# kalj/dealii-cuda

Measured on AMD Instinct MI355X. Metric: DoFs/s on 1305x Laplace vmult (bmop), p=4 3D uniform, higher is better.
Workload: dtype f64; 1 GPU; bmop: DEGREE_FE=4, DIMENSION=3, MATRIX_FREE_UNIFORM_MESH, hyper_cube(-1,1), 54^3 cells, 10218313 DoFs, 1 z-slab(s); cells_per_dir=54, n_dofs=10218313, n_cells=157464, parallelism=slab1, dof_numbering=caller's (lexicographic), finite=True, clock_ramp_steps=2000

## Files before the change

dealii-cuda_amd/csrc/mfgpu_api.hip:

```cpp
#include <hip/hip_runtime.h>

#include <type_traits>

#include <algorithm>
#include <cmath>
#include <cstdlib>
#include <cstring>
#include <memory>
#include <string>
#include <vector>

#include "mfgpu_kernels.h"

using namespace mfgpu;

struct EventTimer {
  std::vector<Event> ev;
  size_t used = 0;
  double ms = 0.0;
  int begin(hipStream_t st) {
    if (used + 2 > ev.size()) {
      Event e0, e1;
      int rc;
      if ((rc = e0.create(hipEventDefault)) || (rc = e1.create(hipEventDefault))) return rc;
// ... 49 lines not shown
  DeviceArray<uint32_t> d_cell_batch, d_cell_pos;
  size_t n_plane_cells = 0;
  DeviceArray<uint32_t> d_cmask, d_orphans;
  DeviceArray<void> d_hnw;
  DeviceArray<uint32_t> d_constrained;
  uint32_t n_constrained = 0;
  DeviceArray<void> d_tabsd;
  DeviceArray<void> d_tab2;
  bool twopass = true;
  DeviceArray<uint32_t> d_batch_nint, d_halo_off;
  std::vector<uint32_t> seg_end;
  std::vector<DeviceArray<uint32_t>> d_p2arr, d_p2tiles;
  std::vector<uint32_t> n_p2tiles;
  DeviceArray<uint32_t> d_p2rec, d_p2tab;
  bool p2_shared = false, p2_reverse = false, no_shared_records = false;
  Stream side;
  std::vector<Event> ev_seg;
  Event ev_side;
  bool side_pending = false;
  DeviceArray<void> d_halo;
  DeviceArray<unsigned long long> d_stamps;
  size_t lds = 0, device_bytes = 0;
  PlaneKernel planes = PlaneKernel::none;
  BatchKernel batches = BatchKernel::none;
  enum { kPlain, kMasked, kBatch };
  CellKernel<double> kernels_f64[3];
  CellKernel<float> kernels_f32[3];
  template <typename T>
  CellKernel<T> &kernel(int which) {
    if constexpr (std::is_same<T, double>::value) return kernels_f64[which];
// ... 61 lines not shown
        const double s = 0.5 * (S[r * n + c] + S[r2 * n + c2]);
        S[r * n + c] = S[r2 * n + c2] = s;
        const double d = 0.5 * (Dt[r * n + c] - Dt[r2 * n + c2]);
        Dt[r * n + c] = d;
        Dt[r2 * n + c2] = -d;
      } else if (r == r2 && c == c2) {
        Dt[r * n + c] = 0.0;
      }
    }
  return 0;
}

int upload_pass2(mfgpu_handle *h, const uint32_t *priority, uint32_t n_priority) {
  const Plan &P = h->plan;
  const size_t ng = 1 + h->seg_end.size();
  const bool shared = P.sh_p2_use && !h->no_shared_records && n_priority == 0 && ng == 2;
  std::vector<Pass2Group> groups;
  int rc;
  if ((rc = pass2_groups(P, h->seg_end, priority, n_priority, shared, groups))) return rc;
  std::vector<DeviceArray<uint32_t>> d_arr(ng), d_tiles(ng);
  std::vector<uint32_t> n_tiles(ng, 0u);
  const bool reverse = (size_t)P.halo_off.back() * esize(h->number_type) <= ((size_t)256 << 20);
  DeviceArray<uint32_t> d_rec, d_tab;
  if (shared) {
    if ((rc = d_rec.upload(P.sh_p2rec.data(), P.sh_p2rec.size()))) return rc;
    if ((rc = d_tab.upload(P.sh_p2tab.data(), P.sh_p2tab.size()))) return rc;
  }
  for (size_t g = 0; g < ng; ++g) {
    std::vector<uint32_t> arr, tiles;
    build_pass2_classes(groups[g].dofs, groups[g].offsets, groups[g].slots, arr, tiles);
    n_tiles[g] = (uint32_t)(tiles.size() / 4);
    if (reverse) {
      const size_t nt = tiles.size() / 4;
      for (size_t a = 0, b = nt ? nt - 1 : 0; a < b; ++a, --b)
        for (int w = 0; w < 4; ++w) std::swap(tiles[4 * a + w], tiles[4 * b + w]);
    }
    if ((rc = d_arr[g].upload(arr.data(), arr.size()))) return rc;
    if ((rc = d_tiles[g].upload(tiles.data(), tiles.size()))) return rc;
  }
  h->d_p2arr = std::move(d_arr);
  h->d_p2tiles = std::move(d_tiles);
// ... 567 lines not shown
  const bool hn = (d.flags & MFGPU_HANGING_NODES) != 0;
  if (hn && (!d.constraint_mask || !d.constraint_weights)) {
    set_error("MFGPU_HANGING_NODES needs constraint_mask and constraint_weights");
    return MFGPU_EINVAL;
  }
  std::unique_ptr<mfgpu_handle, decltype(&mfgpu_destroy)> h(new mfgpu_handle(), mfgpu_destroy);
  int rc = choose_kernel_and_plan(d, h->planes, h->batches, h->plan);
  if (rc) return rc;
  h->dim = d.dim;
  h->n = d.degree + 1;
  h->nd = h->plan.nd;
  h->number_type = d.number_type;
  h->hn = hn;
  h->twopass = !(d.flags & MFGPU_COLORED_SCATTER);
  h->no_shared_records = (d.flags & MFGPU_NO_SHARED_RECORDS) != 0;
  h->updatable = (d.flags & MFGPU_UPDATABLE_COEFFICIENTS) != 0;
  const int nn = h->n * h->n;
  std::vector<double> sv(nn), sg(nn);
  for (int i = 0; i < nn; ++i) {
    sv[i] = d.number_type == MFGPU_F64 ? ((const double *)d.shape_values)[i] : ((const float *)d.shape_values)[i];
    sg[i] = d.number_type == MFGPU_F64 ? ((const double *)d.shape_gradients)[i] : ((const float *)d.shape_gradients)[i];
  }
  h->sv = sv;
  h->sg = sg;
  rc = derive_tables(h->n, sv.data(), sg.data(), h->S, h->Dt);
  if (!rc) rc = check_symmetrize(h->n, h->S, h->Dt);
  if (!rc) rc = d.number_type == MFGPU_F64 ? create_typed<double>(h.get(), d) : create_typed<float>(h.get(), d);
  if (!rc && d.n_constrained) {
    h->n_constrained = d.n_constrained;
    rc = h->d_constrained.upload(d.constrained_dofs, d.n_constrained);
// ... 105 lines not shown
  if (h->twopass) {
    const uint32_t nb = (uint32_t)s[0], npl = P.n_plane_batches, nplain = P.n_plain_plane_batches;
    const uint32_t edge[4] = {0u, nplain, npl, nb};
    s[1] = 0;
    for (size_t g = 0; g < h->seg_end.size(); ++g) {
      const uint32_t s0 = g ? h->seg_end[g - 1] : 0u, s1 = h->seg_end[g];
      for (int f = 0; f < 3; ++f)
        if (std::max(s0, edge[f]) < std::min(s1, edge[f + 1])) ++s[1];
    }
    s[6] = P.sdofs.size();
    s[7] = P.halo_off.back();
  }
  return 0;
}

int mfgpu_record_stats(const mfgpu_handle *h, uint64_t s[4]) {
  if (!h || !s) return MFGPU_EINVAL;
  const Plan &P = h->plan;
  const size_t n = (size_t)P.n, nb = (size_t)p_kgu((int)n) * 64, nx = ((n * n + 1) / 2) * (p_cells_per_wave((int)n) * n);
  const bool planes = h->planes != PlaneKernel::none;
  s[0] = (h->shared_records ? 1 : 0) | (h->p2_shared ? 2 : 0);
  s[1] = planes ? P.sh_dofs.size() / nb : 0;
  s[2] = planes ? P.sh_idx.size() / nx : 0;
  s[3] = h->record_bytes;
  return 0;
}

const char *mfgpu_kernel_name(const mfgpu_handle *h) {
  if (!h) return "";
  const bool x = h->batches == BatchKernel::x;
// ... 149 lines not shown
```

dealii-cuda_amd/csrc/mfgpu_internal.h:

```cpp
#ifndef MFGPU_INTERNAL_H
#define MFGPU_INTERNAL_H

#include <cstdint>
#include <string>
#include <vector>

#include "../../include/mfgpu.h"

namespace mfgpu {

void set_error(const std::string &msg);

inline int ipow(int a, int e) {
  int r = 1;
  for (int i = 0; i < e; ++i) r *= a;
  return r;
}

constexpr int p_cells_per_wave(int n) { return 64 / n; }
constexpr int p_ji(int n) { return n == 3 ? 2 : n == 4 ? 5 : n == 5 ? 9 : n == 6 ? 14 : 23; }
constexpr int p_hs(int n) { return n == 3 ? 3 : n == 4 ? 6 : n == 5 ? 9 : n == 6 ? 14 : 18; }
constexpr int p_kgu(int n) { return p_ji(n) + p_hs(n); }
constexpr int p_cell_stride(int n) {
  int s = n * n * n;
// ... 34 lines not shown
  std::vector<uint32_t> orphans;
  std::vector<uint32_t> batch_nint;
  std::vector<uint32_t> halo_off;
  std::vector<uint32_t> sdofs;
  std::vector<uint32_t> s_off;
  std::vector<uint32_t> s_idx;
  std::vector<uint32_t> chunks;
  std::vector<uint32_t> gstarts;
  uint32_t max_batch_dofs = 0, max_batch_cells = 0;
  uint32_t n_plane_batches = 0;
  uint32_t n_plain_plane_batches = 0;
  std::vector<uint32_t> pr_dofs, pr_idx, pr_hn, pr_hn_slot;
  std::vector<uint32_t> sh_dofs, sh_idx, sh_batch;
  bool sh_use = false;
  std::vector<uint32_t> sh_p2rec, sh_p2tab;
  bool sh_p2_use = false;
  uint64_t n_first = 0, n_add = 0;
};

struct PlanLimits {
  uint32_t max_cells = 0, max_dofs = 0;
  uint32_t interior_max = 0, shared_max = 0, halo_stride = 0;
  bool segregate_masked = false;
  bool masked_planes = false;
  uint32_t private_max = 0;
};

int build_plan(const mfgpu_desc &d, Plan &plan, uint32_t max_chunks = 3, const PlanLimits *limits = nullptr);

struct HnLine {
// ... 17 lines not shown
}
constexpr bool kernel_exists(BatchKernel k, int n, int , bool , bool sh, bool ) {
  return k != BatchKernel::none && n >= 2 && n <= 7 && !sh;
}
constexpr int kFusedWidths[] = {3, 2};
constexpr bool fused_kernel_exists(BatchKernel k, int n, int number_type, bool hn, bool , int nv) {
  return k == BatchKernel::g && n >= 2 && n <= 7 && (nv == 2 || nv == 3) &&
         !(hn && number_type == MFGPU_F64 && n >= (nv == 3 ? 6 : 7));
}
std::vector<uint32_t> multi_groups(uint32_t n_vectors, const std::vector<uint32_t> &widths);
int build_plane_records(Plan &plan, const uint32_t *constraint_mask);
constexpr int kShBatchWords = 4;
constexpr double kShareMaxFraction = 0.5;
void share_plane_records(Plan &plan);
constexpr int kP2Header = 16, kP2MaxK = 12, kP2SlotBits = 12;
void share_pass2_records(Plan &plan);

std::vector<uint16_t> x_lane_permutation(int n);
std::vector<uint16_t> x_pencil_runs(const std::vector<uint16_t> &lmap, int n);
struct Pass2Group {
  std::vector<uint32_t> dofs, offsets = std::vector<uint32_t>(1, 0u), slots;
};
int pass2_groups(const Plan &plan, const std::vector<uint32_t> &seg_end, const uint32_t *priority, uint32_t n_priority,
                 bool shared, std::vector<Pass2Group> &groups);

int derive_tables(int n, const double *shape_values, const double *shape_gradients,
                  std::vector<double> &S, std::vector<double> &Dt);

int handle_number_type(const mfgpu_handle *h);
int handle_set_priority_dofs(mfgpu_handle *h, const uint32_t *ids, uint32_t n);
// ... 20 lines not shown
```

dealii-cuda_amd/csrc/mfgpu_kernels.h:

```cpp
#ifndef MFGPU_KERNELS_H
#define MFGPU_KERNELS_H

#include <hip/hip_runtime.h>

#include <type_traits>

#include "mfgpu_device.h"
#include "mfgpu_internal.h"

namespace mfgpu {

template <typename T>
struct ApplyArgs {
  const uint32_t *batch_cell_off;
  const uint32_t *batch_dof_off;
  const uint32_t *bdofs;
  const uint8_t *bflags;
  const uint16_t *lmap;
  const uint16_t *lmapx;
  const uint16_t *perm;
  const uint32_t *bdofsp;
  const uint32_t *idxp;
  const T *coefp;
  const uint32_t *hnrec;
// ... 106 lines not shown
#undef MFGPU_CELL_LOOP_FAMILY
template <typename T>
using MultiKernel = CellKernel<T, MultiArgs<T>>;
template <typename T, typename Args>
hipError_t g_bind_width(int n, bool hn, bool sh, bool mass, int nv, uint32_t nb_max, CellKernel<T, Args> *k);

void build_pass2_classes(const std::vector<uint32_t> &sdofs, const std::vector<uint32_t> &s_off,
                         const std::vector<uint32_t> &s_idx, std::vector<uint32_t> &arr, std::vector<uint32_t> &tiles);
template <typename T>
hipError_t reduce_classes_launch(T *dst, const T *src, const T *halo, const uint32_t *arr, const uint32_t *tiles,
                                 uint32_t n_tiles, int add, hipStream_t st);
template <typename T>
hipError_t reduce_classes_multi_launch(int nv, T *dst, const T *src, size_t stride, T *const *halos, const uint32_t *arr,
                                       const uint32_t *tiles, uint32_t n_tiles, int add, hipStream_t st);
template <typename T>
hipError_t reduce_owner_batches_launch(T *dst, const T *src, const T *halo, const uint32_t *rec, const uint32_t *tab,
                                       uint32_t n_batches, uint32_t hstride, int reverse, int add, hipStream_t st);
template <typename T>
hipError_t relayout_coef_launch(T *out, const T *in, const uint32_t *cell_batch, const uint32_t *cell_pos,
                                size_t total, int n, hipStream_t st);
template <typename T>
hipError_t fold_general_launch(T *M, const T *coef, const T *jxw, const T *jinv, const uint32_t *order,
                               uint32_t n_cells, uint32_t nd, hipStream_t st);
template <typename T>
hipError_t fold_general2_launch(T *M, const T *coef, const T *jxw, const T *jinv, const uint32_t *order,
                                uint32_t n_cells, uint32_t nd, hipStream_t st);
template <typename T>
hipError_t orphan_launch(T *dst, const T *src, const uint32_t *orph, uint32_t n, int add, hipStream_t st);
template <typename T>
hipError_t coefficient_launch(T *coef, const T *qpts, size_t nq, int dim, hipStream_t st);
template <typename T>
// ... 70 lines not shown
```

dealii-cuda_amd/csrc/mfgpu_pass2.hip:

```cpp
#include <hip/hip_runtime.h>

#include <algorithm>

#include "mfgpu_kernels.h"

namespace mfgpu {

namespace {

template <typename T>
struct GroupHalos {
  size_t stride;
  const T *h[kMaxFusedWidth];
};
template <typename T, typename P>
__device__ __forceinline__ P *vec_at(const T *, P *p, int) { return p; }
template <typename T, typename P>
__device__ __forceinline__ P *vec_at(const GroupHalos<T> &g, P *p, int v) { return p + (size_t)v * g.stride; }
template <typename T>
__device__ __forceinline__ const T *vec_halo(const T *halo, int) { return halo; }
template <typename T>
__device__ __forceinline__ const T *vec_halo(const GroupHalos<T> &g, int v) { return g.h[v]; }

template <typename T, int NV>
// ... 62 lines not shown
reduce_classes(T *__restrict__ dst, const T *__restrict__ src, const HalosArg<T, NV> halos,
               const uint32_t *__restrict__ arr, const uint4 *__restrict__ tiles, int add) {
  const uint4 td = tiles[blockIdx.x];
  const uint32_t *p = arr + td.x;
  const uint32_t i0 = td.w + threadIdx.x;
  switch (td.y) {
    case 1: reduce_two<T, 1, NV>(dst, src, halos, p, td.z, i0, 1, add); break;
    case 2: reduce_two<T, 2, NV>(dst, src, halos, p, td.z, i0, 2, add); break;
    case 3: reduce_two<T, 3, NV>(dst, src, halos, p, td.z, i0, 3, add); break;
    case 4: reduce_two<T, 4, NV>(dst, src, halos, p, td.z, i0, 4, add); break;
    case 8: reduce_two<T, 8, NV>(dst, src, halos, p, td.z, i0, 8, add); break;
    default: reduce_two<T, 0, NV>(dst, src, halos, p, td.z, i0, td.y, add); break;
  }
}

template <typename T, int K>
__device__ __forceinline__ void reduce_owned(T *__restrict__ dst, const T *__restrict__ src,
                                             const T *__restrict__ halo, const uint32_t *__restrict__ r, uint32_t e,
                                             uint32_t d, uint32_t kk, uint32_t kw, uint32_t hslot0, uint32_t hstride,
                                             int add) {
  const T *const hb = halo + hslot0;
  auto partial = [&](uint32_t w) -> T {
    return hb[(w >> kP2SlotBits) * hstride + (w & ((1u << kP2SlotBits) - 1u))];
  };
  constexpr int KU = K > 0 ? K : 1;
  uint32_t w[KU];
#pragma unroll
  for (int t = 0; t < KU; ++t) w[t] = (uint32_t)t < kk ? r[r[3 + t] + e] : 0u;
  if (d == 0xffffffffu) return;
  T v;
  if (d >> 31) {
    v = src[d & 0x7fffffffu];
  } else {
    T q[KU];
#pragma unroll
    for (int t = 0; t < KU; ++t) q[t] = (uint32_t)t < kk ? partial(w[t]) : T(0);
    v = q[0];
#pragma unroll
    for (int t = 1; t < KU; ++t)
      if ((uint32_t)t < kk) v += q[t];
    if (K == 0)
      for (uint32_t t = 1; t < kw; ++t)
        if (t < kk) v += partial(r[r[3 + t] + e]);
  }
  T *const out = dst + (d & 0x7fffffffu);
  *out = add ? *out + v : v;
}

template <typename T>
__global__ void __launch_bounds__(256)
reduce_owner_batches(T *__restrict__ dst, const T *__restrict__ src, const T *__restrict__ halo,
                     const uint32_t *__restrict__ rec, const uint2 *__restrict__ tab, uint32_t n_batches,
                     uint32_t hstride, int reverse, int add) {
  const uint32_t ob = reverse ? n_batches - 1u - blockIdx.x : blockIdx.x;
  const uint2 t = tab[ob];
  const uint32_t *const r = rec + t.y;
  const uint32_t e0 = r[1];
  dst += t.x;
  src += t.x;
  for (uint32_t e = threadIdx.x; e < e0; e += 256u) {
    const uint32_t d = r[kP2Header + e], kk = r[kP2Header + e0 + e];
    const uint32_t kw = (uint32_t)__builtin_amdgcn_readfirstlane((int)kk);
    const uint32_t h0 = ob * hstride;
    switch (kw) {
      case 0: break;
      case 1: reduce_owned<T, 1>(dst, src, halo, r, e, d, kk, kw, h0, hstride, add); break;
      case 2: reduce_owned<T, 2>(dst, src, halo, r, e, d, kk, kw, h0, hstride, add); break;
      case 3: reduce_owned<T, 3>(dst, src, halo, r, e, d, kk, kw, h0, hstride, add); break;
      case 4: reduce_owned<T, 4>(dst, src, halo, r, e, d, kk, kw, h0, hstride, add); break;
      case 5: case 6: case 7:
      case 8: reduce_owned<T, 8>(dst, src, halo, r, e, d, kk, kw, h0, hstride, add); break;
      default: reduce_owned<T, 0>(dst, src, halo, r, e, d, kk, kw, h0, hstride, add); break;
    }
  }
}

}

void build_pass2_classes(const std::vector<uint32_t> &sdofs, const std::vector<uint32_t> &s_off,
                         const std::vector<uint32_t> &s_idx, std::vector<uint32_t> &arr, std::vector<uint32_t> &tiles) {
  arr.clear();
  tiles.clear();
  const size_t ns = sdofs.size();
  uint32_t kmax = 0;
  for (size_t i = 0; i < ns; ++i) kmax = std::max(kmax, s_off[i + 1] - s_off[i]);
  std::vector<std::vector<uint32_t>> members(kmax + 1);
  for (size_t i = 0; i < ns; ++i) {
// ... 37 lines not shown
  GroupHalos<T> gh;
  gh.stride = stride;
  for (int v = 0; v < kMaxFusedWidth; ++v) gh.h[v] = v < nv ? halos[v] : nullptr;
  const uint4 *t4 = reinterpret_cast<const uint4 *>(tiles);
  if (nv == 2)
    hipLaunchKernelGGL((reduce_classes<T, 2>), dim3(n_tiles), dim3(256), 0, st, dst, src, gh, arr, t4, add);
  else
    hipLaunchKernelGGL((reduce_classes<T, 3>), dim3(n_tiles), dim3(256), 0, st, dst, src, gh, arr, t4, add);
  return hipGetLastError();
}
template hipError_t reduce_classes_multi_launch<double>(int, double *, const double *, size_t, double *const *,
                                                        const uint32_t *, const uint32_t *, uint32_t, int, hipStream_t);
template hipError_t reduce_classes_multi_launch<float>(int, float *, const float *, size_t, float *const *,
                                                       const uint32_t *, const uint32_t *, uint32_t, int, hipStream_t);
template <typename T>
hipError_t reduce_owner_batches_launch(T *dst, const T *src, const T *halo, const uint32_t *rec, const uint32_t *tab,
                                       uint32_t n_batches, uint32_t hstride, int reverse, int add, hipStream_t st) {
  if (n_batches == 0) return hipSuccess;
  hipLaunchKernelGGL(reduce_owner_batches<T>, dim3(n_batches), dim3(256), 0, st, dst, src, halo, rec,
                     reinterpret_cast<const uint2 *>(tab), n_batches, hstride, reverse, add);
  return hipGetLastError();
}
template hipError_t reduce_owner_batches_launch<double>(double *, const double *, const double *, const uint32_t *,
                                                        const uint32_t *, uint32_t, uint32_t, int, int, hipStream_t);
template hipError_t reduce_owner_batches_launch<float>(float *, const float *, const float *, const uint32_t *,
                                                       const uint32_t *, uint32_t, uint32_t, int, int, hipStream_t);
template hipError_t reduce_classes_launch<double>(double *, const double *, const double *, const uint32_t *,
                                                  const uint32_t *, uint32_t, int, hipStream_t);
template hipError_t reduce_classes_launch<float>(float *, const float *, const float *, const uint32_t *,
                                                 const uint32_t *, uint32_t, int, hipStream_t);

}
```

dealii-cuda_amd/csrc/mfgpu_plan.cpp:

```cpp
#include <algorithm>
#include <cassert>
#include <cmath>
#include <cstring>
#include <numeric>
#include <unordered_map>

#include "mfgpu_internal.h"

namespace mfgpu {

static thread_local std::string g_err;
void set_error(const std::string &msg) { g_err = msg; }
const char *last_error() { return g_err.c_str(); }

int derive_tables(int n, const double *sv, const double *sg, std::vector<double> &S,
                  std::vector<double> &Dt) {
  std::vector<long double> A(n * n), B(n * n);
  for (int i = 0; i < n * n; ++i) {
    A[i] = sv[i];
    B[i] = sg[i];
  }
  for (int c = 0; c < n; ++c) {
    int piv = c;
    for (int r = c + 1; r < n; ++r)
// ... 849 lines not shown
    for (size_t t = 0; t < NB; ++t) base = std::min(base, g[t] & 0x7fffffffu);
    for (size_t t = 0; t < NB; ++t) rel[t] = g[t] - base;
    uint32_t *e = P.sh_batch.data() + b * kShBatchWords;
    e[0] = base;
    e[1] = (uint32_t)(intern_record(P.sh_dofs, seen_d, rel.data(), NB) / NB);
    e[2] = (uint32_t)(intern_record(P.sh_idx, seen_x, P.pr_idx.data() + b * NX, NX) / NX);
  }
  const size_t shared = P.sh_dofs.size() + P.sh_idx.size() + P.sh_batch.size();
  const size_t expanded = P.pr_dofs.size() + P.pr_idx.size();
  P.sh_use = nbat > 0 && P.pr_hn.empty() && (double)shared <= kShareMaxFraction * (double)expanded;
}

void share_pass2_records(Plan &P) {
  P.sh_p2rec.clear();
  P.sh_p2tab.clear();
  P.sh_p2_use = false;
  const size_t nb = P.batch_cell_off.size() - 1;
  const uint32_t hs = (uint32_t)p_hs(P.n) * 64u;
  if (nb == 0 || P.n_plane_batches != nb || P.halo_off.size() != nb + 1 || hs > (1u << kP2SlotBits)) return;
  for (size_t b = 0; b <= nb; ++b)
    if (P.halo_off[b] != (uint64_t)b * hs) return;
  std::vector<std::vector<uint32_t>> owned(nb);
  size_t expanded = 0;
  for (size_t i = 0; i < P.sdofs.size(); ++i) {
    const uint32_t k = P.s_off[i + 1] - P.s_off[i];
    expanded += 1 + (k ? k : 1);
    if (k == 0) continue;
    if (k > (uint32_t)kP2MaxK) return;
    const uint32_t owner = P.s_idx[P.s_off[i]] / hs;
    for (uint32_t t = 0; t < k; ++t) {
// ... 20 lines not shown
    for (uint32_t e = 0; e < e0; ++e) rec[kP2Header + e] = e < ne ? P.sdofs[m[e]] - base : 0xffffffffu;
    for (uint32_t e = 0; e < ne; ++e) rec[kP2Header + e0 + e] = k_of(m[e]);
    for (uint32_t t = 0; t < kmax; ++t) {
      uint32_t cnt = 0;
      while (cnt < ne && k_of(m[cnt]) > t) ++cnt;
      rec[3 + t] = (uint32_t)rec.size();
      rec.resize(rec.size() + pad(cnt), 0u);
      for (uint32_t e = 0; e < cnt; ++e) {
        const uint32_t slot = P.s_idx[P.s_off[m[e]] + t], tb = slot / hs;
        rec[rec[3 + t] + e] = ((tb - (uint32_t)b) << kP2SlotBits) | (slot - tb * hs);
      }
    }
    P.sh_p2tab[2 * b] = base;
    P.sh_p2tab[2 * b + 1] = (uint32_t)intern_record(P.sh_p2rec, seen, rec.data(), rec.size());
  }
  const size_t shared = P.sh_p2rec.size() + P.sh_p2tab.size();
  P.sh_p2_use = (double)shared <= kShareMaxFraction * (double)expanded;
}

int choose_kernel_and_plan(const mfgpu_desc &d, PlaneKernel &pk, BatchKernel &bk, Plan &plan) {
  const bool general = !(d.flags & MFGPU_UNIFORM_J0), hn = (d.flags & MFGPU_HANGING_NODES) != 0;
  const bool colored = (d.flags & MFGPU_COLORED_SCATTER) != 0;
  if (d.kernel > MFGPU_KERNEL_PLANES_2W) {
    set_error("unknown mfgpu_desc.kernel");
    return MFGPU_EINVAL;
  }
  const bool pk_ok = d.dim == 3 && !general && !colored && d.degree >= 2 && d.degree <= 6 &&
                     d.n_dofs < (1u << 29);
  const bool xk_ok = d.dim == 3 && !general && !colored;
  const bool want_planes = d.kernel == MFGPU_KERNEL_PLANES || d.kernel == MFGPU_KERNEL_PLANES_2W;
  if ((want_planes && !pk_ok) || (d.kernel == MFGPU_KERNEL_PENCILS_X && !xk_ok) ||
// ... 202 lines not shown
    case 7: v = &p->plan.halo_off; break;
    case 8: v = &p->plan.sdofs; break;
    case 9: v = &p->plan.s_off; break;
    case 10: v = &p->plan.s_idx; break;
    case 11: v = &p->plan.chunks; break;
    case 12: v = &p->plan.gstarts; break;
    case 13: v = &p->plan.pr_dofs; break;
    case 14: v = &p->plan.pr_idx; break;
    case 15: v = &p->plan.pr_hn; break;
    case 16: v = &p->plan.pr_hn_slot; break;
    case 17: v = &p->plan.sh_dofs; break;
    case 18: v = &p->plan.sh_idx; break;
    case 19: v = &p->plan.sh_batch; break;
    case 20: v = &p->plan.sh_p2rec; break;
    case 21: v = &p->plan.sh_p2tab; break;
    default: mfgpu::set_error("bad array id"); return MFGPU_EINVAL;
  }
  *ptr = v->data();
  return (int64_t)v->size();
}

int mfgpu_plan_multi_groups(uint32_t n_vectors, const uint32_t *widths, uint32_t n_widths, uint32_t *groups,
                            uint32_t capacity) {
  if ((!widths && n_widths) || (!groups && capacity)) return MFGPU_EINVAL;
  const std::vector<uint32_t> g = mfgpu::multi_groups(n_vectors, std::vector<uint32_t>(widths, widths + n_widths));
  for (size_t i = 0; i < g.size() && i < capacity; ++i) groups[i] = g[i];
  return (int)g.size();
}

int mfgpu_plan_shares_records(const mfgpu_plan *p) {
// ... 17 lines not shown
```

dealii-cuda_amd/pymfgpu/__init__.py:

```python
from __future__ import annotations

import ctypes as C
import os

import numpy as np

_HERE = os.path.dirname(os.path.abspath(__file__))
LIB_PATH = os.environ.get("MFGPU_LIB") or os.path.join(os.path.dirname(_HERE), "lib", "libmfgpu.so")

F64, F32 = 0, 1
OK, EINVAL = 0, -1
EUNSUPPORTED = -4
MULTI_ADD, MULTI_LOOP, MULTI_FUSED = 1, 2, 4
UNIFORM_J0, HANGING_NODES, COLORED_SCATTER, NO_SHARED_RECORDS = 1, 2, 1 << 8, 1 << 9
UPDATABLE_COEFFICIENTS = 1 << 10
KERNEL_AUTO, KERNEL_PENCILS, KERNEL_PENCILS_X, KERNEL_PLANES, KERNEL_PLANES_2W = 0, 1, 2, 3, 4


class MfgpuError(RuntimeError):
    pass


class Desc(C.Structure):
    _fields_ = [
        ("dim", C.c_int32), ("degree", C.c_int32), ("number_type", C.c_int32), ("flags", C.c_uint32),
        ("n_dofs", C.c_uint32), ("n_cells", C.c_uint32),
        ("loc2glob", C.c_void_p), ("constraint_mask", C.c_void_p),
        ("JxW", C.c_void_p), ("inv_jac", C.c_void_p), ("coefficient", C.c_void_p),
        ("quadrature_points", C.c_void_p), ("shape_values", C.c_void_p), ("shape_gradients", C.c_void_p),
# ... 41 lines not shown
                ("n_active", C.c_uint32), ("smoother_degree", C.c_uint32), ("smoothing_range", C.c_double),
                ("eig_iterations", C.c_uint32), ("lambda_max", C.POINTER(C.c_double)), ("coarse", C.c_uint32),
                ("coarse_tolerance", C.c_double), ("coarse_max_iterations", C.c_uint32)]


CG_CALLBACK_TYPE = C.CFUNCTYPE(C.c_int, C.c_void_p, C.c_void_p, C.c_void_p, C.c_void_p)


SYMBOLS = [
    "mfgpu_vmult_multi", "mfgpu_multi_width", "mfgpu_plan_multi_groups",
    "mfgpu_create", "mfgpu_vmult", "mfgpu_vmult_add", "mfgpu_n_dofs", "mfgpu_memory_consumption",
    "mfgpu_destroy", "mfgpu_last_error", "mfgpu_plan_stats", "mfgpu_kernel_name", "mfgpu_compute_inverse_diagonal", "mfgpu_set_constrained_values",
    "mfgpu_vec_sadd", "mfgpu_vec_equ", "mfgpu_vec_scale", "mfgpu_vec_divide", "mfgpu_vec_invert", "mfgpu_vec_mul",
    "mfgpu_vec_dot", "mfgpu_vec_l2_norm", "mfgpu_vec_add_and_dot", "mfgpu_vec_all_zero", "mfgpu_profile_enable", "mfgpu_profile_read", "mfgpu_profile_read_pass2",
    "mfgpu_plan_create", "mfgpu_plan_destroy", "mfgpu_plan_array_u32", "mfgpu_plan_lmap", "mfgpu_plan_bflags",
    "mfgpu_plan_shares_records", "mfgpu_record_stats",
    "mfgpu_vec_alloc", "mfgpu_vec_free", "mfgpu_vec_fill", "mfgpu_vec_from_host", "mfgpu_vec_to_host",
    "mfgpu_device_synchronize", "mfgpu_device_memory_info", "mfgpu_mesh_create_uniform", "mfgpu_mesh_create_adaptive", "mfgpu_mesh_create_ball", "mfgpu_mesh_create_from_leaves",
    "mfgpu_mesh_cell_levels", "mfgpu_mesh_destroy",
    "mfgpu_mesh_desc", "mfgpu_mesh_dof_coords", "mfgpu_mesh_interface_dofs",
    "mfgpu_dist_unique_id", "mfgpu_dist_create", "mfgpu_dist_connect_local", "mfgpu_dist_attach", "mfgpu_dist_schedule",
    "mfgpu_vmult_dist_begin", "mfgpu_vmult_dist_end", "mfgpu_vmult_dist", "mfgpu_dist_destroy",
    "mfgpu_transfer_create", "mfgpu_transfer_create_from_meshes", "mfgpu_transfer_prolongate",
    "mfgpu_transfer_restrict_and_add", "mfgpu_transfer_memory_consumption", "mfgpu_transfer_destroy",
    "mfgpu_mesh_transfer_patches", "mfgpu_suggest_renumbering", "mfgpu_mesh_renumber",
    "mfgpu_level_create", "mfgpu_level_operator", "mfgpu_level_vmult_interface_down", "mfgpu_level_vmult_interface_up",
    "mfgpu_level_destroy", "mfgpu_index_pairs_create", "mfgpu_vec_copy_pairs", "mfgpu_index_pairs_destroy",
    "mfgpu_mesh_create_adaptive_mg", "mfgpu_mg_hierarchy_create", "mfgpu_mg_n_levels", "mfgpu_mg_level_mesh",
    "mfgpu_mg_edge_dofs", "mfgpu_mg_copy_pairs", "mfgpu_mg_transfer_arrays", "mfgpu_mg_hierarchy_destroy",
    "mfgpu_integrator_create", "mfgpu_integrator_rhs", "mfgpu_integrator_l2_error", "mfgpu_integrator_error_points",
    "mfgpu_integrator_destroy",
# ... 56 lines not shown
        L.mfgpu_vec_all_zero.argtypes = [vp, z, i, vp, C.POINTER(i)]
        L.mfgpu_profile_enable.argtypes = [C.c_void_p, C.c_int]
        L.mfgpu_profile_read.argtypes = [C.c_void_p, C.POINTER(C.c_double), C.POINTER(C.c_uint64)]
        L.mfgpu_profile_read_pass2.argtypes = [C.c_void_p, C.POINTER(C.c_double)]
        L.mfgpu_plan_create.argtypes = [C.POINTER(Desc), C.POINTER(C.c_void_p)]
        L.mfgpu_plan_destroy.argtypes = [C.c_void_p]
        L.mfgpu_plan_destroy.restype = None
        L.mfgpu_plan_array_u32.argtypes = [C.c_void_p, C.c_int, C.POINTER(C.c_void_p)]
        L.mfgpu_plan_array_u32.restype = C.c_int64
        L.mfgpu_plan_lmap.argtypes = [C.c_void_p, C.POINTER(C.c_void_p)]
        L.mfgpu_plan_lmap.restype = C.c_int64
        L.mfgpu_plan_bflags.argtypes = [C.c_void_p, C.POINTER(C.c_void_p)]
        L.mfgpu_plan_bflags.restype = C.c_int64
        L.mfgpu_plan_shares_records.argtypes = [C.c_void_p]
        L.mfgpu_record_stats.argtypes = [C.c_void_p, C.POINTER(C.c_uint64)]
        L.mfgpu_vec_alloc.argtypes = [C.POINTER(C.c_void_p), C.c_size_t, C.c_int]
        L.mfgpu_vec_free.argtypes = [C.c_void_p]
        L.mfgpu_vec_fill.argtypes = [C.c_void_p, C.c_size_t, C.c_int, C.c_double, C.c_void_p]
        L.mfgpu_vec_from_host.argtypes = [C.c_void_p, C.c_void_p, C.c_size_t, C.c_int]
        L.mfgpu_vec_to_host.argtypes = [C.c_void_p, C.c_void_p, C.c_size_t, C.c_int]
        L.mfgpu_mesh_create_uniform.argtypes = [C.c_int, C.c_int, C.POINTER(C.c_uint32), C.c_double, C.c_double,
                                                C.c_uint32, C.c_uint32, C.c_int, C.POINTER(C.c_void_p)]
        L.mfgpu_mesh_create_adaptive.argtypes = [C.c_int, C.c_int, C.c_int, C.c_int, C.POINTER(C.c_void_p)]
        L.mfgpu_mesh_create_ball.argtypes = [C.c_int, C.c_int, C.c_int, C.c_int, C.POINTER(C.c_void_p)]
        L.mfgpu_mesh_create_from_leaves.argtypes = [C.c_int, C.c_int, C.c_void_p, C.c_uint32, C.c_int, C.POINTER(C.c_void_p)]
        L.mfgpu_mesh_cell_levels.argtypes = [C.c_void_p, C.POINTER(C.c_void_p)]
        L.mfgpu_mesh_cell_levels.restype = C.c_int64
        L.mfgpu_mesh_destroy.argtypes = [C.c_void_p]
        L.mfgpu_mesh_destroy.restype = None
        L.mfgpu_mesh_desc.argtypes = [C.c_void_p, C.POINTER(Desc)]
# ... 351 lines not shown
    sdofs = property(lambda s: s._u32(8))
    s_off = property(lambda s: s._u32(9))
    s_idx = property(lambda s: s._u32(10))
    chunks = property(lambda s: s._u32(11).reshape(-1, 4))
    gstarts = property(lambda s: s._u32(12))
    pr_dofs = property(lambda s: s._u32(13))
    pr_idx = property(lambda s: s._u32(14))
    pr_hn = property(lambda s: s._u32(15))
    pr_hn_slot = property(lambda s: s._u32(16))
    sh_dofs = property(lambda s: s._u32(17))
    sh_idx = property(lambda s: s._u32(18))
    sh_batch = property(lambda s: s._u32(19).reshape(-1, 4))
    shares_records = property(lambda s: bool(lib().mfgpu_plan_shares_records(s._h) & 1))
    sh_p2rec = property(lambda s: s._u32(20))
    sh_p2tab = property(lambda s: s._u32(21).reshape(-1, 2))
    shares_pass2_records = property(lambda s: bool(lib().mfgpu_plan_shares_records(s._h) & 2))

    @property
    def lmap(self):
        p = C.c_void_p()
        cnt = lib().mfgpu_plan_lmap(self._h, C.byref(p))
        return _view(p.value, cnt, np.uint16).reshape(-1, self.nd).copy()

    @property
    def bflags(self):
        p = C.c_void_p()
        cnt = lib().mfgpu_plan_bflags(self._h, C.byref(p))
        return _view(p.value, cnt, np.uint8).copy()


# ... 119 lines not shown

    def memory_consumption(self):
        return int(lib().mfgpu_memory_consumption(self._h))

    def plan_stats(self):
        s = (C.c_uint64 * 8)()
        _check(lib().mfgpu_plan_stats(self._h, s))
        keys = ["n_batches", "n_launches", "batch_dofs", "max_batch_dofs", "max_batch_cells", "n_orphans",
                "first_touch_or_shared_dofs", "rmw_adds_or_halo_slots"]
        out = dict(zip(keys, [int(v) for v in s]))
        r = (C.c_uint64 * 4)()
        _check(lib().mfgpu_record_stats(self._h, r))
        out.update(index_records="shared" if r[0] & 1 else "expanded",
                   pass2_records="shared" if r[0] & 2 else "expanded", distinct_dof_records=int(r[1]),
                   distinct_index_records=int(r[2]), index_record_bytes=int(r[3]))
        return out

    def kernel_name(self):
        return lib().mfgpu_kernel_name(self._h).decode()

    def compute_inverse_diagonal(self, inv_diag, stream=None):
        _check(lib().mfgpu_compute_inverse_diagonal(self._h, _ptr(inv_diag), stream))

    def set_constrained_values(self, vec, value, stream=None):
        _check(lib().mfgpu_set_constrained_values(self._h, _ptr(vec), float(value), stream))

    def update_coefficients(self, coef=None, mass=None, stream=None):
        _check(lib().mfgpu_update_coefficients(self._h, _optr(coef), _optr(mass), stream))

    def profile_enable(self, on=True):
# ... 698 lines not shown
```

include/mfgpu.h:

```cpp
#ifndef MFGPU_H
#define MFGPU_H

#include <stddef.h>
#include <stdint.h>

#ifdef __cplusplus
extern "C" {
#endif

#define MFGPU_OK 0
#define MFGPU_EINVAL (-1)
#define MFGPU_EHIP (-2)
#define MFGPU_ENOMEM (-3)
#define MFGPU_EUNSUPPORTED (-4)

#define MFGPU_F64 0
#define MFGPU_F32 1

#define MFGPU_UNIFORM_J0 (1u << 0)
#define MFGPU_HANGING_NODES (1u << 1)

#define MFGPU_COLORED_SCATTER (1u << 8)

#define MFGPU_NO_SHARED_RECORDS (1u << 9)

#define MFGPU_UPDATABLE_COEFFICIENTS (1u << 10)

typedef struct mfgpu_handle mfgpu_handle;

typedef struct mfgpu_desc {
  int32_t dim;
  int32_t degree;
  int32_t number_type;
  uint32_t flags;
  uint32_t n_dofs;
  uint32_t n_cells;
  const uint32_t *loc2glob;
  const uint32_t *constraint_mask;
  const void *JxW;
// ... 38 lines not shown

int mfgpu_update_coefficients(mfgpu_handle *h, const void *coefficient_dev, const void *mass_coefficient_dev,
                              void *stream);

uint32_t mfgpu_n_dofs(const mfgpu_handle *h);

size_t mfgpu_memory_consumption(const mfgpu_handle *h);

void mfgpu_destroy(mfgpu_handle *h);

const char *mfgpu_last_error(void);

int mfgpu_plan_stats(const mfgpu_handle *h, uint64_t stats[8]);

int mfgpu_record_stats(const mfgpu_handle *h, uint64_t stats[4]);

const char *mfgpu_kernel_name(const mfgpu_handle *h);

int mfgpu_profile_enable(mfgpu_handle *h, int on);
int mfgpu_profile_read(mfgpu_handle *h, double *kernel_ms_total, uint64_t *n_vmults);
int mfgpu_profile_read_pass2(mfgpu_handle *h, double *pass2_ms_total);

typedef struct mfgpu_plan mfgpu_plan;
int mfgpu_plan_create(const mfgpu_desc *desc, mfgpu_plan **out);
void mfgpu_plan_destroy(mfgpu_plan *p);
int64_t mfgpu_plan_array_u32(const mfgpu_plan *p, int what, const uint32_t **ptr);
int mfgpu_plan_shares_records(const mfgpu_plan *p);
int mfgpu_plan_multi_groups(uint32_t n_vectors, const uint32_t *widths, uint32_t n_widths, uint32_t *groups,
                            uint32_t capacity);
int64_t mfgpu_plan_lmap(const mfgpu_plan *p, const uint16_t **ptr);
// ... 244 lines not shown
```

Measured before the change: 82.21 billion DoFs/s.

## Pack shared pass-2 records and reduce two owner batches per workgroup

Replaces the shared pass-2 record format with a packed entry layout (dof plus two slot words per entry, with a tail region for higher multiplicities) and a 4-word batch table. The owner-batch reduction kernel now processes two owner batches per workgroup and loads partials up front, which removes the runtime switch over multiplicity templates. Flags are added to force record sharing and to choose the traversal order, along with a stats query. The aim is fewer scattered record loads and more memory-level parallelism in the second pass, at the cost of padding, more registers and extra loads for padded lanes.

```diff
diff --git a/dealii-cuda_amd/csrc/mfgpu_api.hip b/dealii-cuda_amd/csrc/mfgpu_api.hip
--- a/dealii-cuda_amd/csrc/mfgpu_api.hip
+++ b/dealii-cuda_amd/csrc/mfgpu_api.hip
@@ -87,6 +87,8 @@
   std::vector<uint32_t> n_p2tiles;
   DeviceArray<uint32_t> d_p2rec, d_p2tab;
   bool p2_shared = false, p2_reverse = false, no_shared_records = false;
+  bool p2_share_always = false;
+  int p2_order = 0;
   Stream side;
   std::vector<Event> ev_seg;
   Event ev_side;
@@ -178,17 +180,19 @@
 int upload_pass2(mfgpu_handle *h, const uint32_t *priority, uint32_t n_priority) {
   const Plan &P = h->plan;
   const size_t ng = 1 + h->seg_end.size();
-  const bool shared = P.sh_p2_use && !h->no_shared_records && n_priority == 0 && ng == 2;
+  const bool shared = (P.sh_p2_use || (h->p2_share_always && !P.sh_p2tab4.empty())) && !h->no_shared_records &&
+                      n_priority == 0 && ng == 2;
   std::vector<Pass2Group> groups;
   int rc;
   if ((rc = pass2_groups(P, h->seg_end, priority, n_priority, shared, groups))) return rc;
   std::vector<DeviceArray<uint32_t>> d_arr(ng), d_tiles(ng);
   std::vector<uint32_t> n_tiles(ng, 0u);
-  const bool reverse = (size_t)P.halo_off.back() * esize(h->number_type) <= ((size_t)256 << 20);
+  const bool reverse = h->p2_order ? h->p2_order < 0
+                                   : (size_t)P.halo_off.back() * esize(h->number_type) <= ((size_t)256 << 20);
   DeviceArray<uint32_t> d_rec, d_tab;
   if (shared) {
-    if ((rc = d_rec.upload(P.sh_p2rec.data(), P.sh_p2rec.size()))) return rc;
-    if ((rc = d_tab.upload(P.sh_p2tab.data(), P.sh_p2tab.size()))) return rc;
+    if ((rc = d_rec.upload(P.sh_p2pk.data(), P.sh_p2pk.size()))) return rc;
+    if ((rc = d_tab.upload(P.sh_p2tab4.data(), P.sh_p2tab4.size()))) return rc;
   }
   for (size_t g = 0; g < ng; ++g) {
     std::vector<uint32_t> arr, tiles;
@@ -786,6 +790,8 @@
   h->hn = hn;
   h->twopass = !(d.flags & MFGPU_COLORED_SCATTER);
   h->no_shared_records = (d.flags & MFGPU_NO_SHARED_RECORDS) != 0;
+  h->p2_share_always = (d.flags & MFGPU_SHARE_PASS2_ALWAYS) != 0;
+  h->p2_order = (d.flags & MFGPU_PASS2_FORWARD) ? 1 : (d.flags & MFGPU_PASS2_REVERSE) ? -1 : 0;
   h->updatable = (d.flags & MFGPU_UPDATABLE_COEFFICIENTS) != 0;
   const int nn = h->n * h->n;
   std::vector<double> sv(nn), sg(nn);
@@ -921,6 +927,15 @@
   return 0;
 }
 
+int mfgpu_pass2_record_stats(const mfgpu_handle *h, uint64_t s[4]) {
+  if (!h || !s) return MFGPU_EINVAL;
+  s[0] = h->p2_shared ? (uint64_t)kP2OwnerBatches : 0;
+  s[1] = h->d_p2rec.bytes();
+  s[2] = h->d_p2tab.bytes();
+  s[3] = h->p2_reverse ? 1 : 0;
+  return 0;
+}
+
 int mfgpu_record_stats(const mfgpu_handle *h, uint64_t s[4]) {
   if (!h || !s) return MFGPU_EINVAL;
   const Plan &P = h->plan;
diff --git a/dealii-cuda_amd/csrc/mfgpu_internal.h b/dealii-cuda_amd/csrc/mfgpu_internal.h
--- a/dealii-cuda_amd/csrc/mfgpu_internal.h
+++ b/dealii-cuda_amd/csrc/mfgpu_internal.h
@@ -72,6 +72,7 @@
   std::vector<uint32_t> sh_dofs, sh_idx, sh_batch;
   bool sh_use = false;
   std::vector<uint32_t> sh_p2rec, sh_p2tab;
+  std::vector<uint32_t> sh_p2pk, sh_p2tab4;
   bool sh_p2_use = false;
   uint64_t n_first = 0, n_add = 0;
 };
@@ -119,6 +120,10 @@
 constexpr double kShareMaxFraction = 0.5;
 void share_plane_records(Plan &plan);
 constexpr int kP2Header = 16, kP2MaxK = 12, kP2SlotBits = 12;
+constexpr int kP2PackedK = 2, kP2EntryWords = 1 + kP2PackedK, kP2PackedPad = kP2EntryWords, kP2OwnerBatches = 2;
+constexpr int kP2UpFrontK = 8;
+constexpr int kP2DofBits = 27;
+static_assert(kP2MaxK < (1 << (31 - kP2DofBits)) - 1, "k must fit its field and leave 0xffffffff to the padding");
 void share_pass2_records(Plan &plan);
 
 std::vector<uint16_t> x_lane_permutation(int n);
diff --git a/dealii-cuda_amd/csrc/mfgpu_kernels.h b/dealii-cuda_amd/csrc/mfgpu_kernels.h
--- a/dealii-cuda_amd/csrc/mfgpu_kernels.h
+++ b/dealii-cuda_amd/csrc/mfgpu_kernels.h
@@ -144,7 +144,7 @@
 hipError_t reduce_classes_multi_launch(int nv, T *dst, const T *src, size_t stride, T *const *halos, const uint32_t *arr,
                                        const uint32_t *tiles, uint32_t n_tiles, int add, hipStream_t st);
 template <typename T>
-hipError_t reduce_owner_batches_launch(T *dst, const T *src, const T *halo, const uint32_t *rec, const uint32_t *tab,
+hipError_t reduce_owner_batches_launch(T *dst, const T *src, const T *halo, const uint32_t *pk, const uint32_t *tab,
                                        uint32_t n_batches, uint32_t hstride, int reverse, int add, hipStream_t st);
 template <typename T>
 hipError_t relayout_coef_launch(T *out, const T *in, const uint32_t *cell_batch, const uint32_t *cell_pos,
diff --git a/dealii-cuda_amd/csrc/mfgpu_pass2.hip b/dealii-cuda_amd/csrc/mfgpu_pass2.hip
--- a/dealii-cuda_amd/csrc/mfgpu_pass2.hip
+++ b/dealii-cuda_amd/csrc/mfgpu_pass2.hip
@@ -100,63 +100,104 @@
   }
 }
 
-template <typename T, int K>
-__device__ __forceinline__ void reduce_owned(T *__restrict__ dst, const T *__restrict__ src,
-                                             const T *__restrict__ halo, const uint32_t *__restrict__ r, uint32_t e,
-                                             uint32_t d, uint32_t kk, uint32_t kw, uint32_t hslot0, uint32_t hstride,
-                                             int add) {
-  const T *const hb = halo + hslot0;
-  auto partial = [&](uint32_t w) -> T {
-    return hb[(w >> kP2SlotBits) * hstride + (w & ((1u << kP2SlotBits) - 1u))];
-  };
-  constexpr int KU = K > 0 ? K : 1;
-  uint32_t w[KU];
-#pragma unroll
-  for (int t = 0; t < KU; ++t) w[t] = (uint32_t)t < kk ? r[r[3 + t] + e] : 0u;
-  if (d == 0xffffffffu) return;
-  T v;
-  if (d >> 31) {
-    v = src[d & 0x7fffffffu];
-  } else {
-    T q[KU];
-#pragma unroll
-    for (int t = 0; t < KU; ++t) q[t] = (uint32_t)t < kk ? partial(w[t]) : T(0);
-    v = q[0];
-#pragma unroll
-    for (int t = 1; t < KU; ++t)
-      if ((uint32_t)t < kk) v += q[t];
-    if (K == 0)
-      for (uint32_t t = 1; t < kw; ++t)
-        if (t < kk) v += partial(r[r[3 + t] + e]);
-  }
-  T *const out = dst + (d & 0x7fffffffu);
-  *out = add ? *out + v : v;
-}
-
-template <typename T>
+struct P2Entry {
+  uint32_t d, w0, w1;
+};
+static_assert(sizeof(P2Entry) == sizeof(uint32_t) * kP2EntryWords, "one packed entry");
+
+template <typename T, int OB>
 __global__ void __launch_bounds__(256)
 reduce_owner_batches(T *__restrict__ dst, const T *__restrict__ src, const T *__restrict__ halo,
-                     const uint32_t *__restrict__ rec, const uint2 *__restrict__ tab, uint32_t n_batches,
+                     const uint32_t *__restrict__ pk, const uint4 *__restrict__ tab, uint32_t n_batches,
                      uint32_t hstride, int reverse, int add) {
-  const uint32_t ob = reverse ? n_batches - 1u - blockIdx.x : blockIdx.x;
-  const uint2 t = tab[ob];
-  const uint32_t *const r = rec + t.y;
-  const uint32_t e0 = r[1];
-  dst += t.x;
-  src += t.x;
-  for (uint32_t e = threadIdx.x; e < e0; e += 256u) {
-    const uint32_t d = r[kP2Header + e], kk = r[kP2Header + e0 + e];
-    const uint32_t kw = (uint32_t)__builtin_amdgcn_readfirstlane((int)kk);
-    const uint32_t h0 = ob * hstride;
-    switch (kw) {
-      case 0: break;
-      case 1: reduce_owned<T, 1>(dst, src, halo, r, e, d, kk, kw, h0, hstride, add); break;
-      case 2: reduce_owned<T, 2>(dst, src, halo, r, e, d, kk, kw, h0, hstride, add); break;
-      case 3: reduce_owned<T, 3>(dst, src, halo, r, e, d, kk, kw, h0, hstride, add); break;
-      case 4: reduce_owned<T, 4>(dst, src, halo, r, e, d, kk, kw, h0, hstride, add); break;
-      case 5: case 6: case 7:
-      case 8: reduce_owned<T, 8>(dst, src, halo, r, e, d, kk, kw, h0, hstride, add); break;
-      default: reduce_owned<T, 0>(dst, src, halo, r, e, d, kk, kw, h0, hstride, add); break;
+  constexpr int KT = kP2UpFrontK - kP2PackedK;
+  constexpr uint32_t slot_mask = (1u << kP2SlotBits) - 1u;
+  uint32_t base[OB], off[OB], e0[OB], e2[OB], km[OB], h0[OB], emax = 0;
+  uint4 t[OB];
+#pragma unroll
+  for (int j = 0; j < OB; ++j) {
+    const uint32_t i = blockIdx.x * OB + j;
+    const uint32_t ob = i < n_batches ? (reverse ? n_batches - 1u - i : i) : 0u;
+    t[j] = tab[ob];
+    h0[j] = ob * hstride;
+  }
+#pragma unroll
+  for (int j = 0; j < OB; ++j) {
+    const bool live = blockIdx.x * OB + j < n_batches;
+    uint32_t tx = t[j].x, ty = t[j].y, tz = t[j].z, tq = t[j].w;
+    asm volatile("" : "+s"(tx), "+s"(ty), "+s"(tz), "+s"(tq));
+    base[j] = tx;
+    off[j] = ty;
+    e0[j] = live ? tz : 0u;
+    e2[j] = live ? tq & 0xffffu : 0u;
+    km[j] = tq >> 16;
+    emax = e0[j] > emax ? e0[j] : emax;
+  }
+  for (uint32_t e = threadIdx.x; e < emax; e += 256u) {
+    const uint32_t ew = (uint32_t)__builtin_amdgcn_readfirstlane((int)e);
+    P2Entry en[OB];
+    bool tail = false;
+#pragma unroll
+    for (int j = 0; j < OB; ++j) {
+      en[j] = *reinterpret_cast<const P2Entry *>(ew < e0[j] ? pk + off[j] + (uint32_t)kP2EntryWords * e : pk);
+      tail |= ew < e2[j];
+    }
+    uint32_t tw[OB][KT];
+#pragma unroll
+    for (int j = 0; j < OB; ++j)
+#pragma unroll
+      for (int t = 0; t < KT; ++t) tw[j][t] = 0u;
+    if (tail) {
+#pragma unroll
+      for (int j = 0; j < OB; ++j) {
+        const bool has = ew < e2[j];
+        const uint32_t rows = km[j] > (uint32_t)kP2PackedK ? km[j] - kP2PackedK : 1u;
+#pragma unroll
+        for (int t = 0; t < KT; ++t) {
+          const uint32_t row = (uint32_t)t < rows ? (uint32_t)t : rows - 1u;
+          tw[j][t] = *(has ? pk + off[j] + (uint32_t)kP2EntryWords * e0[j] + row * e2[j] + e : pk + 1);
+        }
+      }
+    }
+    auto partial = [&](int j, uint32_t w) -> const T * {
+      return halo + h0[j] + ((w >> kP2SlotBits) * hstride + (w & slot_mask));
+    };
+    bool on[OB], sum[OB];
+    uint32_t g[OB];
+    T q0[OB], q1[OB], qt[OB][KT], old[OB];
+#pragma unroll
+    for (int j = 0; j < OB; ++j) {
+      const uint32_t d = en[j].d;
+      on[j] = d != 0xffffffffu;
+      sum[j] = !(d >> 31);
+      g[j] = base[j] + (on[j] ? d & ((1u << kP2DofBits) - 1u) : 0u);
+      q0[j] = *(on[j] && !sum[j] ? src + g[j] : partial(j, en[j].w0));
+      q1[j] = *partial(j, en[j].w1);
+      old[j] = T(0);
+    }
+    if (add) {
+#pragma unroll
+      for (int j = 0; j < OB; ++j) old[j] = dst[g[j]];
+    }
+    if (tail) {
+#pragma unroll
+      for (int j = 0; j < OB; ++j)
+#pragma unroll
+        for (int t = 0; t < KT; ++t) qt[j][t] = *partial(j, tw[j][t]);
+    }
+#pragma unroll
+    for (int j = 0; j < OB; ++j) {
+      const uint32_t kk = sum[j] ? en[j].d >> kP2DofBits : 1u;
+      T v = q0[j];
+      v = kk > 1u ? v + q1[j] : v;
+      if (tail) {
+#pragma unroll
+        for (int t = 0; t < KT; ++t) v = kk > (uint32_t)(kP2PackedK + t) ? v + qt[j][t] : v;
+        if (km[j] > (uint32_t)kP2UpFrontK && ew < e2[j])
+          for (uint32_t t = kP2UpFrontK; t < km[j]; ++t)
+            if (t < kk) v += *partial(j, pk[off[j] + (uint32_t)kP2EntryWords * e0[j] + (t - kP2PackedK) * e2[j] + e]);
+      }
+      if (on[j]) dst[g[j]] = add ? old[j] + v : v;
     }
   }
 }
@@ -224,11 +265,12 @@
 template hipError_t reduce_classes_multi_launch<float>(int, float *, const float *, size_t, float *const *,
                                                        const uint32_t *, const uint32_t *, uint32_t, int, hipStream_t);
 template <typename T>
-hipError_t reduce_owner_batches_launch(T *dst, const T *src, const T *halo, const uint32_t *rec, const uint32_t *tab,
+hipError_t reduce_owner_batches_launch(T *dst, const T *src, const T *halo, const uint32_t *pk, const uint32_t *tab,
                                        uint32_t n_batches, uint32_t hstride, int reverse, int add, hipStream_t st) {
   if (n_batches == 0) return hipSuccess;
-  hipLaunchKernelGGL(reduce_owner_batches<T>, dim3(n_batches), dim3(256), 0, st, dst, src, halo, rec,
-                     reinterpret_cast<const uint2 *>(tab), n_batches, hstride, reverse, add);
+  constexpr uint32_t OB = kP2OwnerBatches;
+  hipLaunchKernelGGL((reduce_owner_batches<T, (int)OB>), dim3((n_batches + OB - 1u) / OB), dim3(256), 0, st, dst, src,
+                     halo, pk, reinterpret_cast<const uint4 *>(tab), n_batches, hstride, reverse, add);
   return hipGetLastError();
 }
 template hipError_t reduce_owner_batches_launch<double>(double *, const double *, const double *, const uint32_t *,
diff --git a/dealii-cuda_amd/csrc/mfgpu_plan.cpp b/dealii-cuda_amd/csrc/mfgpu_plan.cpp
--- a/dealii-cuda_amd/csrc/mfgpu_plan.cpp
+++ b/dealii-cuda_amd/csrc/mfgpu_plan.cpp
@@ -887,6 +887,8 @@
 void share_pass2_records(Plan &P) {
   P.sh_p2rec.clear();
   P.sh_p2tab.clear();
+  P.sh_p2pk.clear();
+  P.sh_p2tab4.clear();
   P.sh_p2_use = false;
   const size_t nb = P.batch_cell_off.size() - 1;
   const uint32_t hs = (uint32_t)p_hs(P.n) * 64u;
@@ -937,7 +939,47 @@
     P.sh_p2tab[2 * b] = base;
     P.sh_p2tab[2 * b + 1] = (uint32_t)intern_record(P.sh_p2rec, seen, rec.data(), rec.size());
   }
-  const size_t shared = P.sh_p2rec.size() + P.sh_p2tab.size();
+  P.sh_p2pk.assign(kP2PackedPad, 0u);
+  P.sh_p2pk[0] = 0xffffffffu;
+  P.sh_p2tab4.assign(4 * nb, 0u);
+  SeenRecords seen_pk;
+  for (size_t b = 0; b < nb; ++b) {
+    const std::vector<uint32_t> &m = owned[b];
+    auto k_of = [&](uint32_t i) { return P.s_off[i + 1] - P.s_off[i]; };
+    auto pad = [](uint32_t x) { return (x + 63u) & ~63u; };
+    const uint32_t ne = (uint32_t)m.size(), kmax = ne ? k_of(m[0]) : 0u, e0 = pad(ne);
+    uint32_t n2 = 0;
+    while (n2 < ne && k_of(m[n2]) > (uint32_t)kP2PackedK) ++n2;
+    const uint32_t e2 = pad(n2);
+    bool fits = e2 < (1u << 16);
+    for (uint32_t e = 0; e < ne; ++e) fits = fits && ((P.sdofs[m[e]] & 0x7fffffffu) - P.sh_p2tab[2 * b]) < (1u << kP2DofBits);
+    if (!fits) {
+      P.sh_p2pk.clear();
+      P.sh_p2tab4.clear();
+      return;
+    }
+    rec.assign(kP2EntryWords * (size_t)e0 + (kmax > (uint32_t)kP2PackedK ? (size_t)(kmax - kP2PackedK) * e2 : 0), 0u);
+    auto word = [&](uint32_t e, uint32_t t) {
+      const uint32_t slot = P.s_idx[P.s_off[m[e]] + t], tb = slot / hs;
+      return ((tb - (uint32_t)b) << kP2SlotBits) | (slot - tb * hs);
+    };
+    for (uint32_t e = 0; e < e0; ++e) {
+      uint32_t *q = rec.data() + kP2EntryWords * (size_t)e;
+      q[0] = 0xffffffffu;
+      if (e >= ne) continue;
+      const uint32_t k = k_of(m[e]);
+      q[0] = (P.sdofs[m[e]] - P.sh_p2tab[2 * b]) | (k << kP2DofBits);
+      for (uint32_t t = 0; t < k; ++t)
+        if (t < (uint32_t)kP2PackedK) q[1 + t] = word(e, t);
+        else rec[kP2EntryWords * (size_t)e0 + (size_t)(t - kP2PackedK) * e2 + e] = word(e, t);
+    }
+    uint32_t *t4 = P.sh_p2tab4.data() + 4 * b;
+    t4[0] = P.sh_p2tab[2 * b];
+    t4[1] = (uint32_t)intern_record(P.sh_p2pk, seen_pk, rec.data(), rec.size());
+    t4[2] = e0;
+    t4[3] = e2 | (kmax << 16);
+  }
+  const size_t shared = P.sh_p2pk.size() + P.sh_p2tab4.size();
   P.sh_p2_use = (double)shared <= kShareMaxFraction * (double)expanded;
 }
 
@@ -1170,6 +1212,8 @@
     case 19: v = &p->plan.sh_batch; break;
     case 20: v = &p->plan.sh_p2rec; break;
     case 21: v = &p->plan.sh_p2tab; break;
+    case 22: v = &p->plan.sh_p2pk; break;
+    case 23: v = &p->plan.sh_p2tab4; break;
     default: mfgpu::set_error("bad array id"); return MFGPU_EINVAL;
   }
   *ptr = v->data();
diff --git a/dealii-cuda_amd/pymfgpu/__init__.py b/dealii-cuda_amd/pymfgpu/__init__.py
--- a/dealii-cuda_amd/pymfgpu/__init__.py
+++ b/dealii-cuda_amd/pymfgpu/__init__.py
@@ -13,6 +13,8 @@
 EUNSUPPORTED = -4
 MULTI_ADD, MULTI_LOOP, MULTI_FUSED = 1, 2, 4
 UNIFORM_J0, HANGING_NODES, COLORED_SCATTER, NO_SHARED_RECORDS = 1, 2, 1 << 8, 1 << 9
+PASS2_FORWARD, PASS2_REVERSE = 1 << 11, 1 << 12
+SHARE_PASS2_ALWAYS = 1 << 13
 UPDATABLE_COEFFICIENTS = 1 << 10
 KERNEL_AUTO, KERNEL_PENCILS, KERNEL_PENCILS_X, KERNEL_PLANES, KERNEL_PLANES_2W = 0, 1, 2, 3, 4
 
@@ -84,7 +86,7 @@
     "mfgpu_vec_sadd", "mfgpu_vec_equ", "mfgpu_vec_scale", "mfgpu_vec_divide", "mfgpu_vec_invert", "mfgpu_vec_mul",
     "mfgpu_vec_dot", "mfgpu_vec_l2_norm", "mfgpu_vec_add_and_dot", "mfgpu_vec_all_zero", "mfgpu_profile_enable", "mfgpu_profile_read", "mfgpu_profile_read_pass2",
     "mfgpu_plan_create", "mfgpu_plan_destroy", "mfgpu_plan_array_u32", "mfgpu_plan_lmap", "mfgpu_plan_bflags",
-    "mfgpu_plan_shares_records", "mfgpu_record_stats",
+    "mfgpu_plan_shares_records", "mfgpu_record_stats", "mfgpu_pass2_record_stats",
     "mfgpu_vec_alloc", "mfgpu_vec_free", "mfgpu_vec_fill", "mfgpu_vec_from_host", "mfgpu_vec_to_host",
     "mfgpu_device_synchronize", "mfgpu_device_memory_info", "mfgpu_mesh_create_uniform", "mfgpu_mesh_create_adaptive", "mfgpu_mesh_create_ball", "mfgpu_mesh_create_from_leaves",
     "mfgpu_mesh_cell_levels", "mfgpu_mesh_destroy",
@@ -171,6 +173,7 @@
         L.mfgpu_plan_bflags.restype = C.c_int64
         L.mfgpu_plan_shares_records.argtypes = [C.c_void_p]
         L.mfgpu_record_stats.argtypes = [C.c_void_p, C.POINTER(C.c_uint64)]
+        L.mfgpu_pass2_record_stats.argtypes = [C.c_void_p, C.POINTER(C.c_uint64)]
         L.mfgpu_vec_alloc.argtypes = [C.POINTER(C.c_void_p), C.c_size_t, C.c_int]
         L.mfgpu_vec_free.argtypes = [C.c_void_p]
         L.mfgpu_vec_fill.argtypes = [C.c_void_p, C.c_size_t, C.c_int, C.c_double, C.c_void_p]
@@ -552,6 +555,8 @@
     shares_records = property(lambda s: bool(lib().mfgpu_plan_shares_records(s._h) & 1))
     sh_p2rec = property(lambda s: s._u32(20))
     sh_p2tab = property(lambda s: s._u32(21).reshape(-1, 2))
+    sh_p2pk = property(lambda s: s._u32(22))
+    sh_p2tab4 = property(lambda s: s._u32(23).reshape(-1, 4))
     shares_pass2_records = property(lambda s: bool(lib().mfgpu_plan_shares_records(s._h) & 2))
 
     @property
@@ -701,6 +706,9 @@
         out.update(index_records="shared" if r[0] & 1 else "expanded",
                    pass2_records="shared" if r[0] & 2 else "expanded", distinct_dof_records=int(r[1]),
                    distinct_index_records=int(r[2]), index_record_bytes=int(r[3]))
+        _check(lib().mfgpu_pass2_record_stats(self._h, r))
+        out.update(pass2_owner_batches_per_workgroup=int(r[0]), pass2_record_bytes=int(r[1]),
+                   pass2_table_bytes=int(r[2]), pass2_reverse=bool(r[3]))
         return out
 
     def kernel_name(self):
diff --git a/include/mfgpu.h b/include/mfgpu.h
--- a/include/mfgpu.h
+++ b/include/mfgpu.h
@@ -23,6 +23,10 @@
 #define MFGPU_COLORED_SCATTER (1u << 8)
 
 #define MFGPU_NO_SHARED_RECORDS (1u << 9)
+
+#define MFGPU_SHARE_PASS2_ALWAYS (1u << 13)
+#define MFGPU_PASS2_FORWARD (1u << 11)
+#define MFGPU_PASS2_REVERSE (1u << 12)
 
 #define MFGPU_UPDATABLE_COEFFICIENTS (1u << 10)
 
@@ -91,6 +95,7 @@
 int mfgpu_plan_stats(const mfgpu_handle *h, uint64_t stats[8]);
 
 int mfgpu_record_stats(const mfgpu_handle *h, uint64_t stats[4]);
+int mfgpu_pass2_record_stats(const mfgpu_handle *h, uint64_t stats[4]);
 
 const char *mfgpu_kernel_name(const mfgpu_handle *h);
 
```

Result: faster. 84.70 billion DoFs/s (median of 6 runs) (+3.0%).
